# 9vvqaq/Indoor-Point-Cloud-Datasets-Controllable-Generation-Method-for-Mobile-Robots-3D-Scene-Perception

Measured on AMD Instinct MI355X. Metric: rays/sec (whole node), 32-line x 2048-azimuth sweep, higher is better.
Workload: dtype f32

## Files before the change

### indoor-point-cloud-datasets-controllable-generation-method-for-mobile-robots-3d-scene-perception_amd/csrc/lidarcast.hip

```cpp
#include <hip/hip_runtime.h>

#include <chrono>
#include <cmath>
#include <cstdio>
#include <cstring>
#include <mutex>
#include <new>
#include <string>
#include <type_traits>
#include <vector>

#include "lrc_internal.h"
#include "lrc_bvh.h"
#include "lrc_qnodes.h"
#include "lrc_device.h"
#include "lrc_gen.h"

using namespace lrcdev;

namespace {
thread_local std::string g_err;
}

int fail(int code, const std::string& msg) {
// ... 705 lines not shown
}

typedef float nt_float4 __attribute__((ext_vector_type(4)));
__device__ __forceinline__ void store_streaming(float4* q, float4 v) {
    const nt_float4 w = {v.x, v.y, v.z, v.w};
    __builtin_nontemporal_store(w, (nt_float4*)q);
}
__device__ __forceinline__ float4 load_streaming(const float4* q) {
    const nt_float4 w = __builtin_nontemporal_load((const nt_float4*)q);
    return make_float4(w.x, w.y, w.z, w.w);
}

template <int R>
__device__ __forceinline__ void scatter_tiles_xyzl_lean(const lrc_compact_io& io, const LeanIn& in, uint64_t ntiles, uint64_t tile0,
                                                        uint32_t lane, const uint32_t* tile_off, const uint32_t* super_total) {
    typedef __attribute__((address_space(4))) const uint64_t cu64;
    typedef __attribute__((address_space(4))) const uint32_t cu32;
    constexpr int H = R < 4 ? R : 4;
    static_assert(R % H == 0, "R: a multiple of four, or below four");
    const uint64_t sbase = super_prefix_wave(super_total, tile0 >> 10, lane);
    const unsigned long long below = (1ull << lane) - 1ull;
#pragma unroll
    for (int h = 0; h < R; h += H) {
        unsigned long long m[H];
        uint32_t off[H];
#pragma unroll
        for (int r = 0; r < H; ++r) {
            const uint64_t tile = tile0 + h + r;
            const bool valid = tile < ntiles;
            m[r] = valid ? ((cu64*)in.keep_mask)[tile] : 0ull;
            off[r] = valid ? ((cu32*)tile_off)[tile] : 0u;
        }
        float4 row[H];
#pragma unroll
        for (int r = 0; r < H; ++r)
            row[r] = m[r] != 0ull ? load_streaming(&in.row[(tile0 + h + r) * 64 + lane]) : make_float4(0.f, 0.f, 0.f, 0.f);
#pragma unroll
        for (int r = 0; r < H; ++r)
            if ((m[r] >> lane) & 1ull)
                store_streaming(&((float4*)io.out_xyzl)[sbase + off[r] + (uint64_t)__popcll(m[r] & below)], row[r]);
    }
}
#ifndef LRC_PRE_TILES
#define LRC_PRE_TILES 8
#endif
constexpr int kPreTiles = LRC_PRE_TILES;

template <int I> struct IntTag { static constexpr int value = I; };

struct alignas(64) RayPose {
    double cx, cy, cz;
    uint32_t same;
    float ox, oy, oz;
    uint32_t pad[6];
};
static_assert(sizeof(RayPose) == 64, "RayPose: four 16-byte units");
constexpr uint64_t kRayTabMaxRows = 1ull << 24;
__host__ __device__ inline uint64_t ray_tab_bytes(uint64_t N, uint64_t P) { return N * 48u + P * sizeof(RayPose); }

__global__ __launch_bounds__(64) void ray_table_kernel(const double* __restrict__ poses16, uint32_t P,
                                                       const double* __restrict__ dirs3, uint32_t N, float4* __restrict__ tab) {
    const uint32_t first = blockIdx.x * 64u + threadIdx.x, step = gridDim.x * 64u;
    const double R[9] = {poses16[0], poses16[1], poses16[2], poses16[4], poses16[5], poses16[6], poses16[8], poses16[9], poses16[10]};
    for (uint32_t i = first; i < N; i += step) {
        const double* dv = dirs3 + (size_t)i * 3;
        const RayRow r = ray_row(R, dv[0], dv[1], dv[2]);
        tab[(size_t)i * 2] = make_float4(r.d.x, r.d.y, r.d.z, 0.0f);
        tab[(size_t)i * 2 + 1] = make_float4(r.inv.x, r.inv.y, r.inv.z, 0.0f);
        tab[(size_t)N * 2 + i] = make_float4(r.h.x, r.h.y, r.h.z, 0.0f);
    }
    RayPose* rp = (RayPose*)(tab + (size_t)N * 3);
    const uint64_t* B = (const uint64_t*)poses16;
    for (uint32_t q = first; q < P; q += step) {
        const double* M = poses16 + (size_t)q * 16;
        const uint64_t* A = (const uint64_t*)M;
        bool same = true;
#pragma unroll
        for (int k = 0; k < 12; ++k)
            if ((k & 3) != 3) same = same & (A[k] == B[k]);
        RayPose o{};
        o.cx = M[3]; o.cy = M[7]; o.cz = M[11];
        o.ox = (float)M[3]; o.oy = (float)M[7]; o.oz = (float)M[11];
        o.same = same ? 1u : 0u;
        rp[q] = o;
    }
}

template <int GEN, int LEAFW, bool UNI, bool SPEC, bool STATS = false, int QN = 0>
__global__ __launch_bounds__(kTBlock, gen_min_waves(GEN, QN, STATS)) void trace_kernel(const TraceParams p) {
    extern __shared__ int s_stack[];
    constexpr bool kCentreFromMotion = gen_centre_from_motion(GEN), kDrawsNoise = gen_draws_noise(GEN);
    const uint32_t tid = threadIdx.x;
    if (GEN == kGenPoses && p.pre.blocks != 0u && p.pre.sharded != 0u) {
        if (blockIdx.x < p.pre.blocks) {
            rebuild_counts(p.pre.rq, blockIdx.x * kTBlock + tid, p.pre.blocks * kTBlock);
            if (blockIdx.x < p.pre.own_blocks) {
                const uint64_t tile0 = (uint64_t)blockIdx.x * kPreTiles;
                if (tile0 < p.pre.ntiles)
                    scatter_tiles_xyzl<kPreTiles>(p.pre.io, p.pre.ntiles, tile0, tid, p.pre.tile_off, nullptr, p.pre.tile_base,
                                                  p.pre.super_base);
            } else {
                const uint32_t tile0 = (blockIdx.x - p.pre.own_blocks) * (uint32_t)LRC_REBUILD_R;
                if (tile0 < p.pre.rq.ntiles) rebuild_tiles<LRC_REBUILD_R>(p.pre.rq, tile0, p.pre.rq.ntiles, tid);
            }
            return;
        }
    } else
    if (GEN == kGenPoses && p.pre.blocks != 0u) {
        if (blockIdx.x < p.pre.blocks) {
            if (p.pre.io.counts) segment_count(p.pre.io, p.pre.tps, p.pre.ntiles, p.pre.nseg, (uint64_t)blockIdx.x * kTBlock + tid,
                                               p.pre.tile_off, nullptr, p.pre.super_total);
            const uint64_t tile0 = (uint64_t)blockIdx.x * kPreTiles;
            if (tile0 < p.pre.ntiles) {
                if (p.pre.rows_only) {
                    scatter_tiles_xyzl_lean<kPreTiles>(p.pre.io, p.pre.lean, p.pre.ntiles, tile0, tid, p.pre.tile_off,
                                                       p.pre.super_total);
                } else {
                    for (int r = 0; r < kPreTiles; ++r)
                        if (tile0 + r < p.pre.ntiles)
                            scatter_tile_lean(p.pre.io, p.pre.lean, p.pre.seg_len, p.pre.tps, tile0 + r, tid, p.pre.tile_off,
                                              p.pre.super_total);
                }
            }
            return;
        }
    }
    const uint32_t tile = p.tile_chunk_log2 ? xcd_tile_chunked(blockIdx.x - p.pre.blocks, gridDim.x - p.pre.blocks, p.tile_chunk_log2)
                                            : xcd_tile(blockIdx.x - p.pre.blocks, gridDim.x - p.pre.blocks);
    const uint64_t gid = (uint64_t)tile * kTBlock + tid;
    if (p.chain_word != nullptr && blockIdx.x == gridDim.x - 1 && tid == 0)
        __hip_atomic_store(p.chain_word, p.chain_seq, __ATOMIC_RELAXED, __HIP_MEMORY_SCOPE_SYSTEM);
    if (gid >= p.total) return;

    V3 o, d;
    V3 inv;
    double cx, cy, cz;
    bool live = true;
    uint32_t pose32 = 0;
    if (GEN == kGenPoses) {
        uint64_t pose, i;
        if (p.tiles_per_pose != 0u) {
            const uint32_t pu = tile / p.tiles_per_pose;
            pose = pu;
            const uint32_t u = tile - pu * p.tiles_per_pose;
            i = p.line_tiles != 0u ? tile_ray(u, tid, p.line_tiles, p.tiles_per_pose, p.line_group) : u * (uint32_t)kTBlock + tid;
        } else {
            pose = gid / p.rays_per_pose;
            i = gid - pose * p.rays_per_pose;
        }
        typedef __attribute__((address_space(4))) const RayPose cpose;
        bool prepared = false;
        if (p.tiles_per_pose != 0u && p.ray_tab != nullptr) {
            cpose* rp = (cpose*)(p.ray_tab + (size_t)p.tiles_per_pose * 192u) + (uint32_t)__builtin_amdgcn_readfirstlane((int)(uint32_t)pose);
            const uint32_t same = rp->same;
            const float ox = rp->ox, oy = rp->oy, oz = rp->oz;
            const float4 ta = p.ray_tab[(size_t)(uint32_t)i * 2], tb = p.ray_tab[(size_t)(uint32_t)i * 2 + 1];
            prepared = same != 0u;
            if (prepared) {
                o.x = ox; o.y = oy; o.z = oz;
                d.x = ta.x; d.y = ta.y; d.z = ta.z;
                inv.x = tb.x; inv.y = tb.y; inv.z = tb.z;
            } else {
                asm volatile("" :: "v"(ta.x), "v"(ta.y), "v"(ta.z), "v"(tb.x), "v"(tb.y), "v"(tb.z), "s"(ox), "s"(oy), "s"(oz));
            }
        }
        if (!prepared) {
            double ux, uy, uz;
            gen_ray(p.poses16, p.dirs3, pose, i, o, d, ux, uy, uz);
            inv = V3{safe_inv(d.x), safe_inv(d.y), safe_inv(d.z)};
        }
        pose32 = (uint32_t)pose;
    } else if (GEN == kGenAngles) {
        const uint64_t pose = gid / p.rays_per_pose;
        const double2 a = ((const double2*)p.angles2)[gid];
        gen_ray_angles(p.poses16, pose, a.x, a.y, o, d, cx, cy, cz);
        if (p.keep_mask) live = p.keep_mask[gid] != 0;
        pose32 = (uint32_t)pose;
    } else if (GEN == kGenSweeps) {
        const uint64_t pose = gid / p.rays_per_pose;
        const uint64_t i = gid - pose * p.rays_per_pose;
        gen_ray_sweep(p.motion24, p.dirs3, p.fire, pose, i, o, d);
        pose32 = (uint32_t)pose;
    } else if (GEN == kGenNoisy) {
        const uint64_t pose = gid / p.rays_per_pose;
        const uint64_t i = gid - pose * p.rays_per_pose;
        gen_ray_noisy(p.poses16, p.dirs3, p.noise, pose, i, o, d, cx, cy, cz, live);
        pose32 = (uint32_t)pose;
    } else if (GEN == kGenNoisySweeps) {
        const uint64_t pose = gid / p.rays_per_pose;
        const uint64_t i = gid - pose * p.rays_per_pose;
        gen_ray_noisy_sweep(p.motion24, p.dirs3, p.fire, p.noise, pose, i, o, d, live);
        pose32 = (uint32_t)pose;
    } else if (GEN == kGenMaterials) {
        const uint64_t pose = gid / p.rays_per_pose;
        double ux, uy, uz;
        gen_ray(p.poses16, p.dirs3, pose, gid - pose * p.rays_per_pose, o, d, ux, uy, uz);
        pose32 = (uint32_t)pose;
    } else if (GEN == kGenEchoes) {
        const uint64_t pose = gid / p.rays_per_pose;
        const uint64_t r = gid - pose * p.rays_per_pose;
        const uint32_t k = tid & ((1u << p.echo.group_log2) - 1u);
        live = k < p.echo.subrays;
        gen_ray_beam(p.poses16, p.dirs3, p.echo.offsets2, pose, r >> p.echo.group_log2, live ? k : 0u, o, d, cx, cy, cz);
        pose32 = (uint32_t)pose;
    } else {
        const float* r = p.rays6 + gid * 6;
        o.x = r[0]; o.y = r[1]; o.z = r[2];
        d.x = r[3]; d.y = r[4]; d.z = r[5];
        if (p.keep_mask) live = p.keep_mask[gid] != 0;
        if (!p.seg_offsets && p.seg_centers3) {
            pose32 = (uint32_t)(gid / p.rays_per_pose);
        } else if (p.seg_offsets) {
            uint32_t lo = 0, hi = p.num_segments;
            while (hi - lo > 1) {
                const uint32_t mid = (lo + hi) >> 1;
                if (p.seg_offsets[mid] <= gid) lo = mid; else hi = mid;
            }
            pose32 = lo;
        }
    }

    float tbest = __builtin_inff();
    uint32_t best_slot = 0xFFFFFFFFu;
    uint32_t best_prim = 0xFFFFFFFFu;
    uint32_t best_label = 0u;

    uint32_t st_nodes = 0, st_tris = 0, st_uni = 0, st_dead = 0, st_pad = 0;
    live = live & finite_ray(o, d);
    if (GEN != kGenPoses) inv = V3{safe_inv(d.x), safe_inv(d.y), safe_inv(d.z)};

    bool redo = false;
    auto traverse = [&](auto qtag, auto ctag) {
        constexpr int QM = decltype(qtag)::value;
        constexpr bool Q = QM != 0;
        constexpr bool INLINE_CLAUSE = decltype(ctag)::value != 0;
        (void)INLINE_CLAUSE;
        RaySlab sl;
        uint32_t sel_nx = 0, sel_ny = 0, sel_nz = 0, sel_fx = 0, sel_fy = 0, sel_fz = 0;
        uint32_t oct = 0;
        if (Q) {
            const float ix = inv.x, iy = inv.y, iz = inv.z;
            sl.ix = ix * p.qW[0]; sl.iy = iy * p.qW[1]; sl.iz = iz * p.qW[2];
            sl.ox = ((o.x - p.qbase[0]) * p.qinvW[0]) * sl.ix;
            sl.oy = ((o.y - p.qbase[1]) * p.qinvW[1]) * sl.iy;
            sl.oz = ((o.z - p.qbase[2]) * p.qinvW[2]) * sl.iz;
            constexpr uint32_t kLo = 0x0701000Cu, kHi = 0x0703020Cu;
            oct = (uint32_t)__builtin_amdgcn_readfirstlane((int)sign_octant(d));
            sel_nx = (oct & 1u) ? kHi : kLo; sel_fx = (oct & 1u) ? kLo : kHi;
            sel_ny = (oct & 2u) ? kHi : kLo; sel_fy = (oct & 2u) ? kLo : kHi;
            sel_nz = (oct & 4u) ? kHi : kLo; sel_fz = (oct & 4u) ? kLo : kHi;
        } else if (INLINE_CLAUSE) {
            V3 dd = d;
            asm volatile("" : "+v"(dd.x), "+v"(dd.y), "+v"(dd.z));
            sl = make_slab(o, dd);
        } else {
            sl.ix = inv.x; sl.iy = inv.y; sl.iz = inv.z;
            sl.ox = o.x * sl.ix; sl.oy = o.y * sl.iy; sl.oz = o.z * sl.iz;
        }
        int sp = 0;
        int ref = 0;
        auto choose = [&](float n0, float f0, float n1, float f1, int r0, int r1) {
            if (STATS) st_nodes += 1u;
            const bool h0 = (n0 <= f0) & (n0 <= tbest);
            const bool h1 = (n1 <= f1) & (n1 <= tbest);
            if (h0 & h1) {
                const bool first0 = n0 <= n1;
                s_stack[sp * kTBlock + tid] = first0 ? r1 : r0;
                ++sp;
                ref = first0 ? r0 : r1;
            } else if (h0) {
                ref = r0;
            } else if (h1) {
                ref = r1;
            } else if (sp == 0) {
                if (STATS) st_dead += 1u;
                ref = ~0;
            } else {
                if (STATS) st_dead += 1u;
                --sp;
                ref = s_stack[sp * kTBlock + tid];
            }
        };
        auto step = [&](const F4 q0, const F4 q1, const F4 q2, const F4 q3) {
            float n0, f0, n1, f1;
            slab_interval(sl, q0.x, q0.y, q0.z, q0.w, q1.x, q1.y, n0, f0);
            slab_interval(sl, q1.z, q1.w, q2.x, q2.y, q2.z, q2.w, n1, f1);
            choose(n0, f0, n1, f1, __float_as_int(q3.x), __float_as_int(q3.y));
        };
        auto step_u = [&](const F4 q0, const F4 q1, const F4 q2, const F4 q3) {
            if (QM == 1) {
                const float c0[6] = {q0.x, q0.y, q0.z, q0.w, q1.x, q1.y}, c1[6] = {q1.z, q1.w, q2.x, q2.y, q2.z, q2.w};
                float n0, f0, n1, f1;
                slab_interval2_oct(sl, oct, c0, c1, n0, f0, n1, f1);
                choose(n0, f0, n1, f1, __float_as_int(q3.x), __float_as_int(q3.y));
            } else {
                step(q0, q1, q2, q3);
            }
        };
        auto step_q = [&](const uint4 a, const uint4 b) {
            auto plane = [](uint32_t w, uint32_t sel) { return __uint_as_float(__builtin_amdgcn_perm(0x40000000u, w, sel)); };
// ... 143 lines not shown
                                    ld_uniform(n + 4), ld_uniform(n + 5), ld_uniform(n + 6), ld_uniform(n + 7));
                        } else
#endif
                        {
                            const float4* n = (Q ? p.nodes_n : p.nodes) + (size_t)uref * 4;
                            step_u(ld_uniform(n), ld_uniform(n + 1), ld_uniform(n + 2), ld_uniform(n + 3));
                        }
                    } else {
                        fetch_step();
                    }
                } else {
                    fetch_step();
                }
                if (SPEC) {
                    if ((ref < 0) & (ref != ~0) & (pending == ~0) & (sp > 0)) {
                        pending = ref;
                        --sp;
                        ref = s_stack[sp * kTBlock + tid];
                    }
                }
            }
            if (SPEC) leaf(pending);
            leaf(ref);
            if (sp == 0) break;
            --sp;
            ref = s_stack[sp * kTBlock + tid];
        }
        if (!INLINE_CLAUSE) {
            if (best_slot != 0xFFFFFFFFu) {
                const float* bx = p.slot_box + (size_t)best_slot * 6;
                best_label = p.slot_label[best_slot];
                RaySlab w = sl;
                if (Q) {
                    w.ix = sl.ix * p.qinvW[0]; w.iy = sl.iy * p.qinvW[1]; w.iz = sl.iz * p.qinvW[2];
                    w.ox = o.x * w.ix; w.oy = o.y * w.iy; w.oz = o.z * w.iz;
                }
                if (!box_clause(w, bx[0], bx[1], bx[2], bx[3], bx[4], bx[5], tbest)) {
                    redo = true;
                    if (STATS) st_pad += 1u;
                }
            }
#ifdef LRC_VARIANTS
            if (p.force_redo) redo |= (((uint64_t)blockIdx.x * kTBlock + tid) % p.force_redo) == 0;
#endif
        }
    };
    using FirstPass = IntTag<0>;
    if (p.num_nodes) {
        if (QN) {
            auto far1 = [](float oa, float da, float base, float W) {
                return !(__builtin_fabsf(oa - base) <= lrc::kQnodeNearBase * W) | !(__builtin_fabsf(oa) <= lrc::kQnodeNearOrigin * W) |
                       !(__builtin_fabsf(da) <= 0x1p60f);
            };
            const bool far = live & (far1(o.x, d.x, p.qbase[0], p.qW[0]) | far1(o.y, d.y, p.qbase[1], p.qW[1]) |
                                     far1(o.z, d.z, p.qbase[2], p.qW[2]));
            const uint32_t oct = sign_octant(d);
            const uint32_t oct0 = (uint32_t)__builtin_amdgcn_readfirstlane((int)oct);
            if (__builtin_amdgcn_ballot_w64(far | (live & (oct != oct0))) != 0ull) { if (live) traverse(IntTag<0>{}, FirstPass{}); }
            else if (live) {
#ifdef LRC_VARIANTS
                if (QN == 2) traverse(IntTag<2>{}, IntTag<0>{});
                else
#endif
                traverse(IntTag<1>{}, IntTag<0>{});
            }
        } else if (live) {
            traverse(IntTag<0>{}, FirstPass{});
        }
        if (__builtin_amdgcn_ballot_w64(redo) != 0ull) {
            if (redo) {
                tbest = __builtin_inff(); best_slot = 0xFFFFFFFFu; best_prim = 0xFFFFFFFFu;
                traverse(IntTag<0>{}, IntTag<1>{});
            }
            best_label = best_slot != 0xFFFFFFFFu ? p.slot_label[best_slot] : 0u;
        }
    }

    const float4* tab = nullptr;
    uint32_t tpp = 0u;
    if (GEN == kGenPoses) {
        tab = p.ray_tab; tpp = p.tiles_per_pose;
        asm volatile("" : "+s"(tab));
        asm volatile("" : "+s"(tpp));
    }
    const bool tabbed = GEN == kGenPoses && tpp != 0u && tab != nullptr;
    if (GEN != kGenRays && !kCentreFromMotion && !tabbed) {
        const double* M = p.poses16;
        asm volatile("" : "+s"(M));
        M += (size_t)pose32 * 16;
        cx = M[3]; cy = M[7]; cz = M[11];
    } else if (GEN != kGenRays) {
    } else if (p.seg_centers3) {
        const double* c = p.seg_centers3 + (size_t)pose32 * 3;
        cx = c[0]; cy = c[1]; cz = c[2];
    } else if (p.has_center) { cx = p.cx; cy = p.cy; cz = p.cz; }
    else { cx = (double)o.x; cy = (double)o.y; cz = (double)o.z; }
    uint32_t wg = blockIdx.x;
    asm volatile("" : "+s"(wg));
    const uint32_t tile_w = p.tile_chunk_log2 ? xcd_tile_chunked(wg - p.pre.blocks, gridDim.x - p.pre.blocks, p.tile_chunk_log2)
                                              : xcd_tile(wg - p.pre.blocks, gridDim.x - p.pre.blocks);
    uint64_t gid_w = (uint64_t)tile_w * kTBlock + tid;
    uint32_t pu_w = 0u;
    if (GEN == kGenPoses && tpp != 0u && (p.line_tiles != 0u || tabbed)) pu_w = tile_w / tpp;
    if (GEN == kGenPoses && tpp != 0u && p.line_tiles != 0u)
        gid_w = (uint64_t)pu_w * p.rays_per_pose + tile_ray(tile_w - pu_w * tpp, tid, p.line_tiles, tpp, p.line_group);
    bool have_h = false;
    V3 h_tab{0.f, 0.f, 0.f};
    if (tabbed) {
        typedef __attribute__((address_space(4))) const RayPose cpose;
        cpose* rp = (cpose*)(tab + (size_t)tpp * 192u) + pu_w;
        const uint32_t same = rp->same;
// ... 314 lines not shown
    rebuild_tiles<R>(q, tile0, q.ntiles, threadIdx.x & 63u);
}

__global__ __launch_bounds__(kBlock) void prim_plane_kernel(const float4* __restrict__ tris, const uint32_t* __restrict__ slot_prim,
                                                            const uint32_t* __restrict__ slot_label, uint32_t num_slots,
                                                            uint32_t num_prims, float4* __restrict__ plane) {
    const uint32_t k = blockIdx.x * kBlock + threadIdx.x;
    if (k >= num_slots) return;
    const uint32_t row = slot_prim[k];
    if (row >= num_prims) return;
    const float4 a = tris[(size_t)k * 3], c = tris[(size_t)k * 3 + 2];
    plane[(size_t)row * 2] = make_float4(a.x, a.y, a.z, __uint_as_float(slot_label[k]));
    plane[(size_t)row * 2 + 1] = make_float4(c.y, c.z, c.w, 0.0f);
}

}

extern "C" {

int lrc_internal_fail(int code, const char* msg) { return fail(code, msg ? msg : ""); }
uint32_t lrc_internal_tile_map(uint64_t line_width, uint32_t tpp, uint32_t* out_ray) {
    const uint32_t wt = line_tiles_for(line_width, (uint64_t)tpp * 64u);
    if (out_ray)
        for (uint32_t u = 0; u < tpp; ++u)
            for (uint32_t l = 0; l < 64u; ++l) out_ray[(size_t)u * 64u + l] = tile_ray(u, l, wt, tpp);
    return wt;
}
uint32_t lrc_internal_tile_map_groups(uint64_t line_width, uint32_t tpp, uint32_t split, uint32_t lines, uint32_t* out_ray) {
    const uint32_t wt = lines >= 2u ? line_tiles_for(line_width, (uint64_t)tpp * 64u) : 0u;
    const uint32_t grp = line_group_for(split, lines);
    if (out_ray)
        for (uint32_t u = 0; u < tpp; ++u)
            for (uint32_t l = 0; l < 64u; ++l) out_ray[(size_t)u * 64u + l] = tile_ray(u, l, wt, tpp, grp);
    return tile_lines_of(wt, tpp, grp);
}
void lrc_internal_range_decide(double max_range, const double* s, uint64_t n, uint8_t* keep, uint8_t* in_band, double* bounds3) {
    const RangeBand rb = range_band(max_range);
    if (bounds3) { bounds3[0] = rb.lo; bounds3[1] = rb.hi; bounds3[2] = (double)rb.fast; }
    for (uint64_t i = 0; i < n; ++i) {
        const bool band = !rb.fast || range_in_band(s[i], rb.lo, rb.hi);
        keep[i] = band ? (uint8_t)(std::sqrt(s[i]) < max_range) : (uint8_t)range_below(s[i], rb.lo);
        if (in_band) in_band[i] = (uint8_t)band;
    }
}

void lrc_internal_ray_table_rows(const double* rot9, const double* dirs3, uint64_t n, float* out9) {
    for (uint64_t i = 0; i < n; ++i) {
        const RayRow r = ray_row(rot9, dirs3[3 * i], dirs3[3 * i + 1], dirs3[3 * i + 2]);
        float* q = out9 + 9 * i;
        q[0] = r.d.x; q[1] = r.d.y; q[2] = r.d.z; q[3] = r.inv.x; q[4] = r.inv.y; q[5] = r.inv.z; q[6] = r.h.x; q[7] = r.h.y; q[8] = r.h.z;
    }
}

const char* lrc_version(void) { return "lidarcast 0.1.0 (gfx950)"; }

const char* lrc_last_error(void) { return g_err.c_str(); }

int lrc_device_count(void) {
    int n = 0;
    if (hipGetDeviceCount(&n) != hipSuccess) { (void)hipGetLastError(); return 0; }
    return n;
}

int lrc_ctx_create(int device, lrc_ctx** out_ctx) {
    if (!out_ctx) return fail(LRC_ERR_INVALID_ARG, "lrc_ctx_create: out_ctx is NULL");
    *out_ctx = nullptr;
    int n = lrc_device_count();
    if (n <= 0) return fail(LRC_ERR_NO_DEVICE, "lrc_ctx_create: no HIP device is visible");
    if (device < 0 || device >= n)
        return fail(LRC_ERR_NO_DEVICE, "lrc_ctx_create: device ordinal out of range");
    LRC_HIP(hipSetDevice(device));
    lrc_ctx* c = new (std::nothrow) lrc_ctx();
    if (!c) return fail(LRC_ERR_OOM, "lrc_ctx_create: out of host memory");
    c->device = device;
    int can_wait = 0;
    if (hipDeviceGetAttribute(&can_wait, hipDeviceAttributeCanUseStreamWaitValue, device) == hipSuccess && can_wait) {
        void* w = nullptr;
        if (hipExtMallocWithFlags(&w, 8, hipMallocSignalMemory) == hipSuccess && w) {
            if (hipStreamWriteValue64(nullptr, w, 0, 0) == hipSuccess && hipStreamSynchronize(nullptr) == hipSuccess) {
                c->chain_word = (uint64_t*)w;
            } else {
                (void)hipFree(w);
            }
        }
    }
    (void)hipGetLastError();
    *out_ctx = c;
    return LRC_OK;
}

int lrc_ctx_set_launch_chaining(lrc_ctx* ctx, int enabled) {
    if (!ctx) return fail(LRC_ERR_INVALID_ARG, "lrc_ctx_set_launch_chaining: ctx is NULL");
    ctx->chain_enabled = enabled != 0;
    return LRC_OK;
}

int lrc_ctx_get_launch_chaining(const lrc_ctx* ctx, int* enabled, int* supported) {
    if (!ctx) return fail(LRC_ERR_INVALID_ARG, "lrc_ctx_get_launch_chaining: ctx is NULL");
    if (enabled) *enabled = ctx->chain_enabled ? 1 : 0;
    if (supported) *supported = ctx->chain_word ? 1 : 0;
    return LRC_OK;
}

int lrc_ctx_destroy(lrc_ctx* ctx) {
    if (!ctx) return LRC_OK;
    (void)hipSetDevice(ctx->device);
// ... 876 lines not shown
    if (nseg == 0 || seg_len == 0) return LRC_OK;
    if (!io->t) return fail(LRC_ERR_INVALID_ARG, "lrc_compact_dev: t is NULL");
    if (((io->out_point3 || io->out_xyzl || io->out_range_origin) && !io->point3) || (io->out_sem && !io->sem) ||
        (io->out_ins && !io->ins) || (io->out_incident_deg && !io->incident_deg))
        return fail(LRC_ERR_INVALID_ARG, "lrc_compact_dev: an output is requested without its input");
    LRC_HIP(hipSetDevice(ctx->device));
    hipStream_t st = (hipStream_t)stream;
    const uint64_t ntiles = nseg * blocks_of(seg_len, 64);
    if (tile_blocks(ntiles) > 0x7FFFFFFFull) return fail(LRC_ERR_INVALID_ARG, "lrc_compact_dev: too many entries");
    int set = -1;
    int rc = compact_scratch_for(ctx, st, ntiles, &set);
    if (rc) return rc;
    if ((rc = enqueue_compaction(ctx->compact_scratch[set], nseg, seg_len, io, st))) return rc;
    LRC_HIP(hipEventRecord(ctx->compact_done[set], st));
    return LRC_OK;
}

#ifndef LRC_PIPE_TILE_LINES
#define LRC_PIPE_TILE_LINES 4
#endif
#ifndef LRC_PIPE_SCAN_WAVES
#define LRC_PIPE_SCAN_WAVES 64
#endif
struct lrc_pipe {
    lrc_scene* scene = nullptr;
    int device = 0;
    uint64_t max_poses = 0, rays_per_pose = 0, cap = 0;
    static constexpr int kSets = 4;
    void* slab[kSets] = {};
    lrc_hits rec[kSets] = {};
    float4* row[kSets] = {};
    uint2* aux[kSets] = {};
    uint64_t* keep_mask[kSets] = {};
    bool lean[kSets] = {};
    bool expanded[kSets] = {};
    lrc_compact_io out[kSets] = {};
    uint64_t poses[kSets] = {};
    bool pending[kSets] = {};
    lrc_ctx::TileScratch scratch[2];
    hipStream_t s_trace[2] = {};
    hipEvent_t ev_in[kSets] = {}, ev_t0[kSets] = {}, ev_trace[kSets] = {}, ev_flush[2] = {}, ev_expand = nullptr;
    bool fused = true;
    uint64_t ticket = 0;
    lrc_ctx::TileScratch gscratch[2];
    uint64_t read_by[kSets] = {};
    uint64_t line_hint = 0;
    const double* line_table = nullptr;
    uint32_t line_auto = 0;
    uint32_t* d_line = nullptr;
    uint32_t line_last = 0;
    uint32_t lines_hint = 0, split_auto = 0, lines_last = 1, group_last = 0;
    float4* ray_tab[2] = {};
    bool use_ray_tab = true;
    bool ray_tab_last = false;
};

int lrc_pipe_destroy(lrc_pipe* pp) {
    if (!pp) return LRC_OK;
    (void)hipSetDevice(pp->device);
    for (hipStream_t st : {pp->s_trace[0], pp->s_trace[1]})
        if (st) { (void)hipStreamSynchronize(st); (void)hipStreamDestroy(st); }
    for (int k = 0; k < lrc_pipe::kSets; ++k) {
        if (pp->slab[k]) (void)hipFree(pp->slab[k]);
        for (hipEvent_t e : {pp->ev_in[k], pp->ev_t0[k], pp->ev_trace[k]}) if (e) (void)hipEventDestroy(e);
    }
    if (pp->ev_expand) (void)hipEventDestroy(pp->ev_expand);
    if (pp->d_line) (void)hipFree(pp->d_line);
    for (int k = 0; k < 2; ++k) {
        if (pp->ray_tab[k]) (void)hipFree(pp->ray_tab[k]);
        if (pp->ev_flush[k]) (void)hipEventDestroy(pp->ev_flush[k]);
        pp->scratch[k].release();
        pp->gscratch[k].release();
    }
    delete pp;
    return LRC_OK;
}

int lrc_pipe_create(lrc_scene* s, uint64_t max_poses, uint64_t rays_per_pose, lrc_pipe** out_pipe) {
    if (!out_pipe) return fail(LRC_ERR_INVALID_ARG, "lrc_pipe_create: out_pipe is NULL");
    *out_pipe = nullptr;
    if (!s) return fail(LRC_ERR_INVALID_ARG, "lrc_pipe_create: scene is NULL");
    if (max_poses == 0 || rays_per_pose == 0) return fail(LRC_ERR_INVALID_ARG, "lrc_pipe_create: max_poses and rays_per_pose must be positive");
    if (max_poses > 0x7FFFFFFFull || max_poses * rays_per_pose / rays_per_pose != max_poses || max_poses * rays_per_pose > (1ull << 36))
        return fail(LRC_ERR_INVALID_ARG, "lrc_pipe_create: batch too large");
    LRC_HIP(hipSetDevice(s->ctx->device));
    lrc_pipe* pp = new (std::nothrow) lrc_pipe();
    if (!pp) return fail(LRC_ERR_OOM, "lrc_pipe_create: out of host memory");
    pp->scene = s;
    pp->device = s->ctx->device;
    pp->max_poses = max_poses;
    pp->rays_per_pose = rays_per_pose;
    const uint64_t n = pp->cap = max_poses * rays_per_pose;
    const uint64_t tiles = max_poses * blocks_of(rays_per_pose, 64);
    pp->fused = rays_per_pose % 64 == 0 && blocks_of(tiles, 1024) <= 512;
    auto bail = [&](int rc) { (void)lrc_pipe_destroy(pp); return rc; };
    auto up = [](uint64_t b) { return (b + 255) & ~255ull; };
    const uint64_t off_t = 0, off_prim = off_t + up(4 * n), off_nrm = off_prim + up(4 * n), off_pt = off_nrm + up(12 * n),
                   off_sem = off_pt + up(12 * n), off_ins = off_sem + up(2 * n), off_tc = off_ins + up(2 * n),
                   off_row = off_tc + up(4 * ((n + 63) / 64)), off_aux = off_row + (pp->fused ? up(16 * n) : 0),
                   off_km = off_aux + (pp->fused ? up(8 * n) : 0), bytes = off_km + (pp->fused ? up(8 * ((n + 63) / 64)) : 0);
    for (int k = 0; k < lrc_pipe::kSets; ++k) {
        hipError_t e = hipMalloc(&pp->slab[k], bytes);
        if (e != hipSuccess) { (void)hipGetLastError(); return bail(fail(LRC_ERR_OOM, "lrc_pipe_create: out of device memory for the record sets")); }
        char* b = (char*)pp->slab[k];
        lrc_hits& h = pp->rec[k];
        h.t = (float*)(b + off_t); h.prim = (uint32_t*)(b + off_prim); h.normal3 = (float*)(b + off_nrm);
        h.point3 = (float*)(b + off_pt); h.sem = (uint16_t*)(b + off_sem); h.ins = (uint16_t*)(b + off_ins);
        h.tile_count = (uint32_t*)(b + off_tc);
        if (pp->fused) {
            pp->row[k] = (float4*)(b + off_row); pp->aux[k] = (uint2*)(b + off_aux); pp->keep_mask[k] = (uint64_t*)(b + off_km);
        }
    }
    int prio_least = 0, prio_greatest = 0;
    if (hipDeviceGetStreamPriorityRange(&prio_least, &prio_greatest) != hipSuccess) return bail(fail(LRC_ERR_HIP, "lrc_pipe_create: stream priorities"));
    for (int k = 0; k < 2; ++k) {
        if (hipStreamCreateWithPriority(&pp->s_trace[k], hipStreamNonBlocking, prio_least) != hipSuccess) return bail(fail(LRC_ERR_HIP, "lrc_pipe_create: stream"));
        if (hipEventCreateWithFlags(&pp->ev_flush[k], hipEventDisableTiming) != hipSuccess) return bail(fail(LRC_ERR_HIP, "lrc_pipe_create: event"));
        int rc = ensure_tile_scratch(pp->scratch[k], tiles);
        if (rc) return bail(rc);
    }
    for (int k = 0; k < lrc_pipe::kSets; ++k) {
        if (hipEventCreateWithFlags(&pp->ev_in[k], hipEventDisableTiming) != hipSuccess ||
            hipEventCreate(&pp->ev_t0[k]) != hipSuccess || hipEventCreate(&pp->ev_trace[k]) != hipSuccess)
            return bail(fail(LRC_ERR_HIP, "lrc_pipe_create: event"));
    }
    if (hipEventCreateWithFlags(&pp->ev_expand, hipEventDisableTiming) != hipSuccess) return bail(fail(LRC_ERR_HIP, "lrc_pipe_create: event"));
    if (pp->fused && hipMalloc((void**)&pp->d_line, 2 * sizeof(uint32_t)) != hipSuccess) { (void)hipGetLastError(); return bail(fail(LRC_ERR_OOM, "lrc_pipe_create: out of device memory")); }
    if (pp->fused && kTBlock == 64 && rays_per_pose <= kRayTabMaxRows)
        for (int k = 0; k < 2; ++k)
            if (hipMalloc((void**)&pp->ray_tab[k], ray_tab_bytes(rays_per_pose, max_poses)) != hipSuccess) { (void)hipGetLastError(); return bail(fail(LRC_ERR_OOM, "lrc_pipe_create: out of device memory for the ray tables")); }
    *out_pipe = pp;
    return LRC_OK;
}

}

namespace {
lrc_compact_io pipe_io(const lrc_pipe* pp, int set) {
    lrc_compact_io io = pp->out[set];
    const lrc_hits& h = pp->rec[set];
    io.t = h.t; io.point3 = h.point3; io.sem = h.sem; io.ins = h.ins; io.incident_deg = nullptr; io.tile_count = h.tile_count;
    return io;
}
LeanIn pipe_lean(const lrc_pipe* pp, int set) {
    if (!pp->lean[set]) return LeanIn{nullptr, nullptr};
    return LeanIn{pp->row[set], pp->keep_mask[set]};
}
int wait_for_readers(lrc_pipe* pp, int set, hipStream_t T) {
    const uint64_t r = pp->read_by[set];
    if (r != 0 && pp->s_trace[(r - 1) % 2] != T) LRC_HIP(hipStreamWaitEvent(T, pp->ev_trace[(r - 1) % lrc_pipe::kSets], 0));
    pp->read_by[set] = 0;
    return LRC_OK;
}
}

extern "C" {

uint32_t lrc_internal_pipe_line_tiles(const lrc_pipe* pp) { return pp ? pp->line_last : 0u; }

uint32_t lrc_internal_pipe_tile_lines(const lrc_pipe* pp) { return pp ? pp->lines_last : 0u; }
uint32_t lrc_internal_pipe_line_group(const lrc_pipe* pp) { return pp ? pp->group_last : 0u; }

int lrc_pipe_set_tile_lines(lrc_pipe* pp, uint32_t lines) {
    if (!pp) return fail(LRC_ERR_INVALID_ARG, "lrc_pipe_set_tile_lines: pipe is NULL");
    if (lines != 0u && lines != 1u && lines != 2u && lines != 4u) return fail(LRC_ERR_INVALID_ARG, "lrc_pipe_set_tile_lines: lines must be 0, 1, 2 or 4");
    pp->lines_hint = lines;
    return LRC_OK;
}

int lrc_pipe_set_ray_table(lrc_pipe* pp, int enable) {
    if (!pp) return fail(LRC_ERR_INVALID_ARG, "lrc_pipe_set_ray_table: pipe is NULL");
    if (enable != 0 && enable != 1) return fail(LRC_ERR_INVALID_ARG, "lrc_pipe_set_ray_table: enable must be 0 or 1");
    pp->use_ray_tab = enable != 0;
    return LRC_OK;
}

const void* lrc_internal_pipe_ray_table(const lrc_pipe* pp) {
    return pp && pp->ray_tab_last ? (const void*)pp->ray_tab[(pp->ticket - 1) % 2] : nullptr;
}

int lrc_pipe_set_line_width(lrc_pipe* pp, uint64_t line_width) {
    if (!pp) return fail(LRC_ERR_INVALID_ARG, "lrc_pipe_set_line_width: pipe is NULL");
    pp->line_hint = line_width;
    pp->line_table = nullptr;
    return LRC_OK;
}

int lrc_pipe_submit(lrc_pipe* pp, const double* d_poses16, uint64_t P, const double* d_dirs3, double max_range,
                    const lrc_compact_io* d_out, void* stream, uint64_t* out_ticket) {
    if (!pp || !d_out) return fail(LRC_ERR_INVALID_ARG, "lrc_pipe_submit: NULL pipe or output");
    if (P == 0) { if (out_ticket) *out_ticket = pp->ticket; return LRC_OK; }
    if (P > pp->max_poses) return fail(LRC_ERR_INVALID_ARG, "lrc_pipe_submit: more poses than the pipeline was created for");
    if (!d_poses16 || !d_dirs3) return fail(LRC_ERR_INVALID_ARG, "lrc_pipe_submit: poses16 or dirs3 is NULL");
    if (d_out->out_incident_deg) return fail(LRC_ERR_INVALID_ARG, "lrc_pipe_submit: the pipeline's records carry no incident angle");
    lrc_scene* s = pp->scene;
    LRC_HIP(hipSetDevice(s->ctx->device));
    const uint64_t k = pp->ticket;
    const int set = (int)(k % lrc_pipe::kSets), lane = (int)(k % 2);
    hipStream_t T = pp->s_trace[lane];
    LRC_HIP(hipEventRecord(pp->ev_in[set], (hipStream_t)stream));
    LRC_HIP(hipStreamWaitEvent(T, pp->ev_in[set], 0));
    int rc = wait_for_readers(pp, set, T);
    if (rc) return rc;
    const uint64_t N = pp->rays_per_pose;
    TraceParams p{};
    p.poses16 = d_poses16;
    p.dirs3 = d_dirs3;
    scan_fields(p, N, P * N, max_range, &pp->rec[set]);
    if (pp->fused) {
        p.lean.row = pp->row[set]; p.lean.aux = pp->aux[set]; p.lean.keep_mask = pp->keep_mask[set];
        if (pp->line_hint == 0 && pp->line_table != d_dirs3) {
            uint32_t w[2] = {0, 0};
            hipLaunchKernelGGL(first_line_kernel, dim3(1), dim3(64), 0, (hipStream_t)stream, d_dirs3, N, pp->d_line);
            LRC_HIP(hipGetLastError());
            LRC_HIP(hipMemcpyAsync(w, pp->d_line, sizeof(w), hipMemcpyDeviceToHost, (hipStream_t)stream));
            LRC_HIP(hipStreamSynchronize((hipStream_t)stream));
            pp->line_auto = line_tiles_for(w[0], N);
            pp->split_auto = w[1];
            pp->line_table = d_dirs3;
        }
        p.line_tiles = kTBlock == 64 && pp->lines_hint != 1u ? (pp->line_hint ? line_tiles_for(pp->line_hint, N) : pp->line_auto) : 0u;
        if (p.line_tiles != 0u)
            p.line_group = line_group_for(pp->line_hint == 0 ? pp->split_auto : 0u,
                                          pp->lines_hint == 0u ? (uint32_t)LRC_PIPE_TILE_LINES : pp->lines_hint);
    }
    pp->ray_tab_last = false;
    if (pp->fused && pp->use_ray_tab && pp->ray_tab[lane]) {
        const uint64_t rows = N > P ? N : P, waves = blocks_of(rows, 64);
        hipLaunchKernelGGL(ray_table_kernel, dim3((uint32_t)(waves < 64 ? waves : 64)), dim3(64), 0, T, d_poses16, (uint32_t)P, d_dirs3,
                           (uint32_t)N, pp->ray_tab[lane]);
        LRC_HIP(hipGetLastError());
        p.ray_tab = pp->ray_tab[lane];
        pp->ray_tab_last = true;
    }
    const int prev = (int)((k + lrc_pipe::kSets - 2) % lrc_pipe::kSets);
    lrc_compact_io pio{};
    if (pp->fused && k >= 2 && pp->pending[prev]) {
        pio = pipe_io(pp, prev);
        const uint64_t tps = N / 64, ntiles = pp->poses[prev] * tps;
        const uint64_t need = pio.counts ? blocks_of(pp->poses[prev], kTBlock) : 0;
        const uint64_t pre_blocks = blocks_of(ntiles, kPreTiles);
        p.pre.blocks = (uint32_t)(pre_blocks > need ? pre_blocks : need);
        p.pre.rows_only = (pio.out_xyzl && !pio.out_point3 && !pio.out_sem && !pio.out_ins && !pio.out_index && !pio.out_range_origin) ? 1u : 0u;
        p.pre.seg_len = N; p.pre.tps = tps; p.pre.ntiles = ntiles; p.pre.nseg = pp->poses[prev];
        p.pre.tile_off = pp->scratch[lane].d_tile_off;
        p.pre.super_total = pp->scratch[lane].d_super_total;
        p.pre.io = pio;
        p.pre.lean = pipe_lean(pp, prev);
    }
    LRC_HIP(hipEventRecord(pp->ev_t0[set], T));
    rc = launch_trace(s, p, kGenPoses, T);
    if (rc) return rc;
    LRC_HIP(hipEventRecord(pp->ev_trace[set], T));
    pp->line_last = p.line_tiles;
    pp->group_last = p.line_group;
    pp->lines_last = tile_lines_of(p.line_tiles, (uint32_t)(N / 64), p.line_group);
    if (p.pre.blocks) pp->pending[prev] = false;
    pp->out[set] = *d_out;
    pp->poses[set] = P;
    pp->lean[set] = p.lean.row != nullptr;
    pp->expanded[set] = false;
    if (pp->fused) {
        const uint64_t ntiles = P * (N / 64), nsuper = blocks_of(ntiles, 1024);
        hipLaunchKernelGGL(compact_scan_masks_kernel, dim3((uint32_t)(nsuper < LRC_PIPE_SCAN_WAVES ? nsuper : LRC_PIPE_SCAN_WAVES)), dim3(64), 0, T,
                           (const uint64_t*)pp->keep_mask[set], pp->rec[set].tile_count, pp->scratch[lane].d_tile_off, ntiles,
                           pp->scratch[lane].d_super_total);
        LRC_HIP(hipGetLastError());
        pp->pending[set] = true;
    } else {
        lrc_compact_io io = pipe_io(pp, set);
        rc = enqueue_compaction(pp->scratch[lane], P, N, &io, T);
        if (rc) return rc;
    }
    pp->ticket = k + 1;
    if (out_ticket) *out_ticket = k + 1;
    return LRC_OK;
}

}

namespace {
int check_gathered(const lrc_pipe* pp, const lrc_gathered* g, const char* who, uint64_t max_back) {
    auto bad = [&](const char* m) { return fail(LRC_ERR_INVALID_ARG, std::string(who) + ": " + m); };
// ... 1429 lines not shown
```

### indoor-point-cloud-datasets-controllable-generation-method-for-mobile-robots-3d-scene-perception_amd/csrc/lrc_device.h

```cpp
#pragma once
#include <hip/hip_runtime.h>
#include <stdint.h>

#include "lrc_noise.h"

namespace lrcdev {

#define LRC_DI __device__ __forceinline__
#define LRC_HDI __host__ __device__ __forceinline__

constexpr float kTinyDir = 1e-30f;
constexpr float kPadRelLo = 0.999755859375f;
constexpr float kPadRelHi = 1.000244140625f;
constexpr float kPadAbs   = 1.52587890625e-05f;
constexpr double kRadToDeg = 57.29577951308232;

struct V3 { float x, y, z; };

LRC_DI float fma_(float a, float b, float c) { return __builtin_fmaf(a, b, c); }
LRC_DI float dot3(V3 a, V3 b) { return fma_(a.z, b.z, fma_(a.y, b.y, a.x * b.x)); }
LRC_DI V3 cross3(V3 a, V3 b) {
    V3 r;
    r.x = fma_(a.y, b.z, -(a.z * b.y));
    r.y = fma_(a.z, b.x, -(a.x * b.z));
// ... 209 lines not shown
    const double ux = s * M[13], uy = s * M[14], uz = s * M[15];
    const double n = ((qw * qw + ux * ux) + uy * uy) + uz * uz;
    const double kk = 2.0 / n;
    const double tx = uy * vz - uz * vy, ty = uz * vx - ux * vz, tz = ux * vy - uy * vx;
    const double wx = uy * tz - uz * ty, wy = uz * tx - ux * tz, wz = ux * ty - uy * tx;
    d.x = (float)(vx + kk * (qw * tx + wx));
    d.y = (float)(vy + kk * (qw * ty + wy));
    d.z = (float)(vz + kk * (qw * tz + wz));
    double cx, cy, cz;
    sweep_centre(M, s, cx, cy, cz);
    o.x = (float)cx; o.y = (float)cy; o.z = (float)cz;
}

LRC_DI void gen_ray_beam(const double* poses16, const double* dirs3, const double* offsets2, uint64_t pose, uint64_t i,
                         uint32_t k, V3& o, V3& d, double& cx, double& cy, double& cz) {
    const double* M = poses16 + pose * 16;
    const double* dv = dirs3 + i * 3;
    double a = dv[0], b = dv[1], c = dv[2];
    const double du = offsets2[2 * k], dt = offsets2[2 * k + 1];
    if (du != 0.0 || dt != 0.0) {
        const double h = __builtin_sqrt(a * a + b * b);
        if (h != 0.0) {
            const double dp = du / h;
            lrcnoise::jitter_row(a, b, c, dp, dt);
        }
    }
    d.x = (float)dgemm_row(a, b, c, M[0], M[1], M[2]);
    d.y = (float)dgemm_row(a, b, c, M[4], M[5], M[6]);
    d.z = (float)dgemm_row(a, b, c, M[8], M[9], M[10]);
    cx = M[3]; cy = M[7]; cz = M[11];
    o.x = (float)cx; o.y = (float)cy; o.z = (float)cz;
}

LRC_HDI V3 unit_dir(V3 d) {
    const float nrm = __builtin_sqrtf((d.x * d.x + d.y * d.y) + d.z * d.z);
    return V3{d.x / nrm, d.y / nrm, d.z / nrm};
}
LRC_DI void hit_point(V3 o, V3 d, float t, V3& h, V3& pt) {
    h = unit_dir(d);
    pt.x = o.x + h.x * t; pt.y = o.y + h.y * t; pt.z = o.z + h.z * t;
}

struct RayRow { V3 d, inv, h; };
LRC_HDI RayRow ray_row(const double* R, double a, double b, double c) {
    RayRow r;
    r.d.x = (float)dgemm_row(a, b, c, R[0], R[1], R[2]);
    r.d.y = (float)dgemm_row(a, b, c, R[3], R[4], R[5]);
    r.d.z = (float)dgemm_row(a, b, c, R[6], R[7], R[8]);
    r.inv = V3{safe_inv(r.d.x), safe_inv(r.d.y), safe_inv(r.d.z)};
    r.h = unit_dir(r.d);
    return r;
}

LRC_HDI uint32_t tile_ray(uint32_t u, uint32_t lane, uint32_t wt, uint32_t tpp, uint32_t grp = 0u) {
    if (wt == 0u) return u * 64u + lane;
    const uint32_t line = u / wt, c = u - line * wt;
    const uint32_t s = grp & 0x7FFFFFFFu;
    const uint64_t sw = (uint64_t)s * wt;
    const uint32_t l0 = line < s ? 0u : s;
    const uint32_t lim = (line < s && sw < tpp) ? (uint32_t)sw : tpp;
    const uint32_t k = line - l0;
    const uint32_t b4 = (grp >> 31) != 0u ? (k & ~3u) : 0u;
    if ((grp >> 31) != 0u && (l0 + b4 + 4u) * wt <= lim)
        return ((l0 + b4 + (lane >> 4)) * wt) * 64u + ((k & 3u) * wt + c) * 16u + (lane & 15u);
    const uint32_t b2 = b4 + ((k - b4) & ~1u);
    if ((l0 + b2 + 2u) * wt <= lim)
        return ((l0 + b2 + (lane >> 5)) * wt) * 64u + (((k - b4) & 1u) * wt + c) * 32u + (lane & 31u);
    return u * 64u + lane;
}
LRC_HDI uint32_t line_group_for(uint32_t split, uint32_t lines) {
    return (split > 0x7FFFFFFFu ? 0u : split) | (lines == 4u ? 0x80000000u : 0u);
}
LRC_HDI uint32_t tile_lines_of(uint32_t wt, uint32_t tpp, uint32_t grp) {
    if (wt == 0u) return 1u;
    const uint32_t hf = tpp / wt;
    uint32_t s = grp & 0x7FFFFFFFu;
    if (s >= hf) s = 0u;
    const uint32_t a = s, b = hf - s, m = a > b ? a : b;
    return ((grp >> 31) != 0u && m >= 4u) ? 4u : (m >= 2u ? 2u : 1u);
}
LRC_HDI uint32_t line_tiles_for(uint64_t W, uint64_t N) {
    if (W == 0 || W % 64u != 0 || N % W != 0 || N / W < 2u || N > 0xFFFFFFFFull) return 0u;
    return (uint32_t)(W / 64u);
}

struct RangeBand { double lo, hi; int fast; };
LRC_HDI RangeBand range_band(double R) {
    RangeBand b{0.0, 0.0, 0};
    if (!(R >= 0x1p-500) || !(R <= 0x1p500)) return b;
    const double r2 = R * R;
    b.lo = r2 * (1.0 - 0x1p-48);
    b.hi = r2 * (1.0 + 0x1p-48);
    b.fast = 1;
    return b;
}
LRC_HDI bool range_in_band(double s, double lo, double hi) { return (s >= lo) & (s <= hi); }
LRC_HDI bool range_below(double s, double lo) { return s < lo; }

}
```

Baseline: 15.56 billion.

## Precompute per-tile quantised-traversal eligibility and octant in ray table

The ray-table kernel now also computes, for each 64-ray tile, whether every ray is finite and shares one sign octant, and for each pose whether its origin lies near the quantised grid. It also stores the pose origin already normalised to that grid. The trace kernel reads these scalar records and skips the per-ray far test, the octant ballot, the finite-ray check and the origin normalisation when both flags hold. This trims per-ray setup and wave-wide ballots at the cost of extra scalar loads, a slightly larger table allocation offset before the base pointer, and more work in the table kernel.

```diff
diff --git a/indoor-point-cloud-datasets-controllable-generation-method-for-mobile-robots-3d-scene-perception_amd/csrc/lidarcast.hip b/indoor-point-cloud-datasets-controllable-generation-method-for-mobile-robots-3d-scene-perception_amd/csrc/lidarcast.hip
--- a/indoor-point-cloud-datasets-controllable-generation-method-for-mobile-robots-3d-scene-perception_amd/csrc/lidarcast.hip
+++ b/indoor-point-cloud-datasets-controllable-generation-method-for-mobile-robots-3d-scene-perception_amd/csrc/lidarcast.hip
@@ -781,16 +781,49 @@
     double cx, cy, cz;
     uint32_t same;
     float ox, oy, oz;
-    uint32_t pad[6];
+    uint32_t near;
+    float nox, noy, noz;
+    uint32_t pad[2];
 };
 static_assert(sizeof(RayPose) == 64, "RayPose: four 16-byte units");
+struct alignas(16) TileRec {
+    uint32_t quant;
+    uint32_t oct;
+    uint32_t pad[2];
+};
+static_assert(sizeof(TileRec) == 16, "TileRec: one 16-byte unit");
+__host__ __device__ inline uint32_t ray_tab_front(uint32_t tiles_per_pose) { return (tiles_per_pose + 3u) & ~3u; }
+__device__ __forceinline__ TileRec tile_rec_wave(V3 d) {
+    const TileRow r = tile_row(d);
+    const uint32_t oct0 = (uint32_t)__builtin_amdgcn_readfirstlane((int)r.oct);
+    const bool all = __builtin_amdgcn_ballot_w64(!r.ok | (r.oct != oct0)) == 0ull;
+    return TileRec{all ? 1u : 0u, oct0, {0u, 0u}};
+}
+__device__ __forceinline__ bool pose_near(float oa, float base, float W) {
+    return (__builtin_fabsf(oa - base) <= lrc::kQnodeNearBase * W) & (__builtin_fabsf(oa) <= lrc::kQnodeNearOrigin * W);
+}
+struct RayTabGrid { float qbase[3], qW[3], qinvW[3]; uint32_t quantised; };
 constexpr uint64_t kRayTabMaxRows = 1ull << 24;
 __host__ __device__ inline uint64_t ray_tab_bytes(uint64_t N, uint64_t P) { return N * 48u + P * sizeof(RayPose); }
 
 __global__ __launch_bounds__(64) void ray_table_kernel(const double* __restrict__ poses16, uint32_t P,
-                                                       const double* __restrict__ dirs3, uint32_t N, float4* __restrict__ tab) {
-    const uint32_t first = blockIdx.x * 64u + threadIdx.x, step = gridDim.x * 64u;
+                                                       const double* __restrict__ dirs3, uint32_t N, float4* __restrict__ tab,
+                                                       const RayTabGrid g, uint32_t tile_recs, uint32_t wt, uint32_t grp,
+                                                       uint32_t row_blocks) {
+    const uint32_t first = blockIdx.x * 64u + threadIdx.x, step = row_blocks * 64u;
     const double R[9] = {poses16[0], poses16[1], poses16[2], poses16[4], poses16[5], poses16[6], poses16[8], poses16[9], poses16[10]};
+    const uint32_t tpp = N / 64u;
+    TileRec* trec = (TileRec*)tab - ray_tab_front(tpp);
+    if (blockIdx.x >= row_blocks) {
+        for (uint32_t u = blockIdx.x - row_blocks; u < tpp; u += gridDim.x - row_blocks) {
+            const uint32_t row = tile_ray(u, threadIdx.x, wt, tpp, grp);
+            const double* dv = dirs3 + (size_t)(row < N ? row : N - 1u) * 3;
+            TileRec t = tile_rec_wave(ray_row(R, dv[0], dv[1], dv[2]).d);
+            if (tile_recs == 0u) t.quant = 0u;
+            if (threadIdx.x == 0) trec[u] = t;
+        }
+        return;
+    }
     for (uint32_t i = first; i < N; i += step) {
         const double* dv = dirs3 + (size_t)i * 3;
         const RayRow r = ray_row(R, dv[0], dv[1], dv[2]);
@@ -811,6 +844,13 @@
         o.cx = M[3]; o.cy = M[7]; o.cz = M[11];
         o.ox = (float)M[3]; o.oy = (float)M[7]; o.oz = (float)M[11];
         o.same = same ? 1u : 0u;
+        const uint32_t m = 0x7F800000u;
+        const bool fin = ((__float_as_uint(o.ox) & m) != m) & ((__float_as_uint(o.oy) & m) != m) & ((__float_as_uint(o.oz) & m) != m);
+        o.near = (tile_recs != 0u && g.quantised != 0u && fin && pose_near(o.ox, g.qbase[0], g.qW[0]) &&
+                  pose_near(o.oy, g.qbase[1], g.qW[1]) && pose_near(o.oz, g.qbase[2], g.qW[2])) ? 1u : 0u;
+        o.nox = (o.ox - g.qbase[0]) * g.qinvW[0];
+        o.noy = (o.oy - g.qbase[1]) * g.qinvW[1];
+        o.noz = (o.oz - g.qbase[2]) * g.qinvW[2];
         rp[q] = o;
     }
 }
@@ -866,6 +906,9 @@
     double cx, cy, cz;
     bool live = true;
     uint32_t pose32 = 0;
+    bool rec_quant = false;
+    uint32_t rec_oct = 0u;
+    V3 rec_no{0.f, 0.f, 0.f};
     if (GEN == kGenPoses) {
         uint64_t pose, i;
         if (p.tiles_per_pose != 0u) {
@@ -880,17 +923,29 @@
         typedef __attribute__((address_space(4))) const RayPose cpose;
         bool prepared = false;
         if (p.tiles_per_pose != 0u && p.ray_tab != nullptr) {
-            cpose* rp = (cpose*)(p.ray_tab + (size_t)p.tiles_per_pose * 192u) + (uint32_t)__builtin_amdgcn_readfirstlane((int)(uint32_t)pose);
+            typedef __attribute__((address_space(4))) const TileRec ctile;
+            const uint32_t pu = (uint32_t)__builtin_amdgcn_readfirstlane((int)(uint32_t)pose);
+            cpose* rp = (cpose*)(p.ray_tab + (size_t)p.tiles_per_pose * 192u) + pu;
+            ctile* tr = (ctile*)p.ray_tab - ray_tab_front(p.tiles_per_pose) + (tile - pu * p.tiles_per_pose);
             const uint32_t same = rp->same;
             const float ox = rp->ox, oy = rp->oy, oz = rp->oz;
+            const uint32_t near = rp->near;
+            const float nox = rp->nox, noy = rp->noy, noz = rp->noz;
+            const uint32_t tq = tr->quant, toct = tr->oct;
             const float4 ta = p.ray_tab[(size_t)(uint32_t)i * 2], tb = p.ray_tab[(size_t)(uint32_t)i * 2 + 1];
             prepared = same != 0u;
             if (prepared) {
                 o.x = ox; o.y = oy; o.z = oz;
                 d.x = ta.x; d.y = ta.y; d.z = ta.z;
                 inv.x = tb.x; inv.y = tb.y; inv.z = tb.z;
+                if (QN == 1) {
+                    rec_quant = (near & tq) != 0u;
+                    rec_oct = toct;
+                    rec_no = V3{nox, noy, noz};
+                }
             } else {
-                asm volatile("" :: "v"(ta.x), "v"(ta.y), "v"(ta.z), "v"(tb.x), "v"(tb.y), "v"(tb.z), "s"(ox), "s"(oy), "s"(oz));
+                asm volatile("" :: "v"(ta.x), "v"(ta.y), "v"(ta.z), "v"(tb.x), "v"(tb.y), "v"(tb.z), "s"(ox), "s"(oy), "s"(oz),
+                             "s"(near), "s"(nox), "s"(noy), "s"(noz), "s"(tq), "s"(toct));
             }
         }
         if (!prepared) {
@@ -955,9 +1010,10 @@
     uint32_t best_label = 0u;
 
     uint32_t st_nodes = 0, st_tris = 0, st_uni = 0, st_dead = 0, st_pad = 0;
-    live = live & finite_ray(o, d);
+    if (__builtin_expect(!rec_quant, 1)) live = live & finite_ray(o, d);
     if (GEN != kGenPoses) inv = V3{safe_inv(d.x), safe_inv(d.y), safe_inv(d.z)};
 
+    uint32_t q_oct = 0u;
     bool redo = false;
     auto traverse = [&](auto qtag, auto ctag) {
         constexpr int QM = decltype(qtag)::value;
@@ -970,11 +1026,15 @@
         if (Q) {
             const float ix = inv.x, iy = inv.y, iz = inv.z;
             sl.ix = ix * p.qW[0]; sl.iy = iy * p.qW[1]; sl.iz = iz * p.qW[2];
-            sl.ox = ((o.x - p.qbase[0]) * p.qinvW[0]) * sl.ix;
-            sl.oy = ((o.y - p.qbase[1]) * p.qinvW[1]) * sl.iy;
-            sl.oz = ((o.z - p.qbase[2]) * p.qinvW[2]) * sl.iz;
+            if (rec_quant) {
+                sl.ox = rec_no.x * sl.ix; sl.oy = rec_no.y * sl.iy; sl.oz = rec_no.z * sl.iz;
+            } else {
+                sl.ox = ((o.x - p.qbase[0]) * p.qinvW[0]) * sl.ix;
+                sl.oy = ((o.y - p.qbase[1]) * p.qinvW[1]) * sl.iy;
+                sl.oz = ((o.z - p.qbase[2]) * p.qinvW[2]) * sl.iz;
+            }
             constexpr uint32_t kLo = 0x0701000Cu, kHi = 0x0703020Cu;
-            oct = (uint32_t)__builtin_amdgcn_readfirstlane((int)sign_octant(d));
+            oct = q_oct;
             sel_nx = (oct & 1u) ? kHi : kLo; sel_fx = (oct & 1u) ? kLo : kHi;
             sel_ny = (oct & 2u) ? kHi : kLo; sel_fy = (oct & 2u) ? kLo : kHi;
             sel_nz = (oct & 4u) ? kHi : kLo; sel_fz = (oct & 4u) ? kLo : kHi;
@@ -1224,11 +1284,17 @@
                 return !(__builtin_fabsf(oa - base) <= lrc::kQnodeNearBase * W) | !(__builtin_fabsf(oa) <= lrc::kQnodeNearOrigin * W) |
                        !(__builtin_fabsf(da) <= 0x1p60f);
             };
-            const bool far = live & (far1(o.x, d.x, p.qbase[0], p.qW[0]) | far1(o.y, d.y, p.qbase[1], p.qW[1]) |
-                                     far1(o.z, d.z, p.qbase[2], p.qW[2]));
-            const uint32_t oct = sign_octant(d);
-            const uint32_t oct0 = (uint32_t)__builtin_amdgcn_readfirstlane((int)oct);
-            if (__builtin_amdgcn_ballot_w64(far | (live & (oct != oct0))) != 0ull) { if (live) traverse(IntTag<0>{}, FirstPass{}); }
+            bool quant = true;
+            if (__builtin_expect(rec_quant, 0)) {
+                q_oct = rec_oct;
+            } else {
+                const bool far = live & (far1(o.x, d.x, p.qbase[0], p.qW[0]) | far1(o.y, d.y, p.qbase[1], p.qW[1]) |
+                                         far1(o.z, d.z, p.qbase[2], p.qW[2]));
+                const uint32_t oct = sign_octant(d);
+                q_oct = (uint32_t)__builtin_amdgcn_readfirstlane((int)oct);
+                quant = __builtin_amdgcn_ballot_w64(far | (live & (oct != q_oct))) == 0ull;
+            }
+            if (!quant) { if (live) traverse(IntTag<0>{}, FirstPass{}); }
             else if (live) {
 #ifdef LRC_VARIANTS
                 if (QN == 2) traverse(IntTag<2>{}, IntTag<0>{});
@@ -1649,6 +1715,22 @@
     }
 }
 
+void lrc_internal_tile_records(const double* rot9, const double* dirs3, uint64_t n, uint32_t wt, uint32_t grp, uint32_t* out2) {
+    const uint32_t tpp = (uint32_t)(n / 64);
+    for (uint32_t u = 0; u < tpp; ++u) {
+        bool all = true;
+        uint32_t oct0 = 0u;
+        for (uint32_t l = 0; l < 64u; ++l) {
+            const uint64_t i = tile_ray(u, l, wt, tpp, grp);
+            const TileRow r = tile_row(ray_row(rot9, dirs3[3 * i], dirs3[3 * i + 1], dirs3[3 * i + 2]).d);
+            if (l == 0u) oct0 = r.oct;
+            all = all && r.ok && r.oct == oct0;
+        }
+        out2[2 * u] = all ? 1u : 0u;
+        out2[2 * u + 1] = oct0;
+    }
+}
+
 const char* lrc_version(void) { return "lidarcast 0.1.0 (gfx950)"; }
 
 const char* lrc_last_error(void) { return g_err.c_str(); }
@@ -2631,6 +2713,7 @@
     uint32_t lines_hint = 0, split_auto = 0, lines_last = 1, group_last = 0;
     float4* ray_tab[2] = {};
     bool use_ray_tab = true;
+    bool use_tile_recs = true;
     bool ray_tab_last = false;
 };
 
@@ -2646,7 +2729,7 @@
     if (pp->ev_expand) (void)hipEventDestroy(pp->ev_expand);
     if (pp->d_line) (void)hipFree(pp->d_line);
     for (int k = 0; k < 2; ++k) {
-        if (pp->ray_tab[k]) (void)hipFree(pp->ray_tab[k]);
+        if (pp->ray_tab[k]) (void)hipFree(pp->ray_tab[k] - ray_tab_front((uint32_t)(pp->rays_per_pose / 64)));
         if (pp->ev_flush[k]) (void)hipEventDestroy(pp->ev_flush[k]);
         pp->scratch[k].release();
         pp->gscratch[k].release();
@@ -2706,8 +2789,12 @@
     if (hipEventCreateWithFlags(&pp->ev_expand, hipEventDisableTiming) != hipSuccess) return bail(fail(LRC_ERR_HIP, "lrc_pipe_create: event"));
     if (pp->fused && hipMalloc((void**)&pp->d_line, 2 * sizeof(uint32_t)) != hipSuccess) { (void)hipGetLastError(); return bail(fail(LRC_ERR_OOM, "lrc_pipe_create: out of device memory")); }
     if (pp->fused && kTBlock == 64 && rays_per_pose <= kRayTabMaxRows)
-        for (int k = 0; k < 2; ++k)
-            if (hipMalloc((void**)&pp->ray_tab[k], ray_tab_bytes(rays_per_pose, max_poses)) != hipSuccess) { (void)hipGetLastError(); return bail(fail(LRC_ERR_OOM, "lrc_pipe_create: out of device memory for the ray tables")); }
+        for (int k = 0; k < 2; ++k) {
+            const uint32_t front = ray_tab_front((uint32_t)(rays_per_pose / 64));
+            float4* base = nullptr;
+            if (hipMalloc((void**)&base, (uint64_t)front * sizeof(TileRec) + ray_tab_bytes(rays_per_pose, max_poses)) != hipSuccess) { (void)hipGetLastError(); return bail(fail(LRC_ERR_OOM, "lrc_pipe_create: out of device memory for the ray tables")); }
+            pp->ray_tab[k] = base + front;
+        }
     *out_pipe = pp;
     return LRC_OK;
 }
@@ -2756,6 +2843,16 @@
 
 const void* lrc_internal_pipe_ray_table(const lrc_pipe* pp) {
     return pp && pp->ray_tab_last ? (const void*)pp->ray_tab[(pp->ticket - 1) % 2] : nullptr;
+}
+
+int lrc_internal_pipe_set_tile_records(lrc_pipe* pp, int enable) {
+    if (!pp) return fail(LRC_ERR_INVALID_ARG, "lrc_internal_pipe_set_tile_records: pipe is NULL");
+    pp->use_tile_recs = enable != 0;
+    return LRC_OK;
+}
+
+const void* lrc_internal_pipe_tile_records(const lrc_pipe* pp) {
+    return pp && pp->ray_tab_last ? (const void*)(pp->ray_tab[(pp->ticket - 1) % 2] - ray_tab_front((uint32_t)(pp->rays_per_pose / 64))) : nullptr;
 }
 
 int lrc_pipe_set_line_width(lrc_pipe* pp, uint64_t line_width) {
@@ -2806,8 +2903,12 @@
     pp->ray_tab_last = false;
     if (pp->fused && pp->use_ray_tab && pp->ray_tab[lane]) {
         const uint64_t rows = N > P ? N : P, waves = blocks_of(rows, 64);
-        hipLaunchKernelGGL(ray_table_kernel, dim3((uint32_t)(waves < 64 ? waves : 64)), dim3(64), 0, T, d_poses16, (uint32_t)P, d_dirs3,
-                           (uint32_t)N, pp->ray_tab[lane]);
+        RayTabGrid g{};
+        for (int a = 0; a < 3; ++a) { g.qbase[a] = s->qbase[a]; g.qW[a] = s->qW[a]; g.qinvW[a] = s->qinvW[a]; }
+        g.quantised = s->d_nodes_q != nullptr ? 1u : 0u;
+        const uint32_t row_blocks = (uint32_t)(waves < 64 ? waves : 64), tile_blocks = (uint32_t)(N / 64 < 64 ? N / 64 : 64);
+        hipLaunchKernelGGL(ray_table_kernel, dim3(row_blocks + tile_blocks), dim3(64), 0, T, d_poses16, (uint32_t)P, d_dirs3,
+                           (uint32_t)N, pp->ray_tab[lane], g, pp->use_tile_recs ? 1u : 0u, p.line_tiles, p.line_group, row_blocks);
         LRC_HIP(hipGetLastError());
         p.ray_tab = pp->ray_tab[lane];
         pp->ray_tab_last = true;
diff --git a/indoor-point-cloud-datasets-controllable-generation-method-for-mobile-robots-3d-scene-perception_amd/csrc/lrc_device.h b/indoor-point-cloud-datasets-controllable-generation-method-for-mobile-robots-3d-scene-perception_amd/csrc/lrc_device.h
--- a/indoor-point-cloud-datasets-controllable-generation-method-for-mobile-robots-3d-scene-perception_amd/csrc/lrc_device.h
+++ b/indoor-point-cloud-datasets-controllable-generation-method-for-mobile-robots-3d-scene-perception_amd/csrc/lrc_device.h
@@ -285,6 +285,17 @@
     return r;
 }
 
+struct TileRow { bool ok; uint32_t oct; };
+LRC_HDI TileRow tile_row(V3 d) {
+    const uint32_t m = 0x7F800000u;
+    const uint32_t bx = __builtin_bit_cast(uint32_t, d.x), by = __builtin_bit_cast(uint32_t, d.y), bz = __builtin_bit_cast(uint32_t, d.z);
+    TileRow r;
+    r.ok = ((bx & m) != m) & ((by & m) != m) & ((bz & m) != m) &
+           (__builtin_fabsf(d.x) <= 0x1p60f) & (__builtin_fabsf(d.y) <= 0x1p60f) & (__builtin_fabsf(d.z) <= 0x1p60f);
+    r.oct = (bx >> 31) | ((by >> 31) << 1) | ((bz >> 31) << 2);
+    return r;
+}
+
 LRC_HDI uint32_t tile_ray(uint32_t u, uint32_t lane, uint32_t wt, uint32_t tpp, uint32_t grp = 0u) {
     if (wt == 0u) return u * 64u + lane;
     const uint32_t line = u / wt, c = u - line * wt;
```

Result: no change. 15.64 billion (median of 6 runs) (+0.5%).
